# KristinnVikarJ/nbody-simulation

Measured on AMD Instinct MI355X. Metric: pair-interactions/sec + ms/step at N=1M direct O(N^2) (force + integration step), higher is better.
Workload: dtype f32; 1 GPU; direct O(N^2) f32, N=1048576 bodies, seeded 2-D Plummer sphere, masses 1, dt=0.1, clamp=0.001 (BASELINE.json configs[2]); n_bodies=1048576, targets_per_gpu=1048576, n_ranks=1, entry=one process per GPU (sharding.py over nbody_direct_{prep,run}_dev), exchange=none, arith=AUTO (FAST kernel; EXACT on hazardous positions)

## Files before the change

### nbody-simulation_amd/csrc/direct_kernels.h

```cpp
#pragma once
#include <hip/hip_runtime.h>
#include <stddef.h>
#include <stdint.h>

namespace nbody {

enum { kFlagHazard = 0, kFlagFallback = 1, kFlagNearCount = 2, kFlagState = 3 };

struct DirectArgs {
  const float2* pos_all;
  const float2* src_pos;
  const float* mass_all;
  int n_src;
  int tgt_begin;
  int n_tgt;
  float2* vel;
  float2* pos_out;
  float2* acc_out;
  float2* partial;
  int to_partial;
  float delta;
  float clamp;
  float uniform_mass;
  const int* flags;
  int run_state;
  const uint32_t* near_list;
  int src_couples;
  const float* src_minv;
  const float* tile_mass;
};

struct DirectConfig {
  int tpt = 1;
  int gsplit = 1;
  int use_asm = 4;
  bool nearfar = true;
};

struct NearFarLayout {
  size_t table_keys, table_bytes, is_near, scan, near_list, pos_far, minv_far, cub_temp, cub_temp_bytes, total;
};
NearFarLayout nearfar_layout(int64_t n_src);
constexpr int64_t kMaxMassClasses = 32;
constexpr int64_t kDirectTile = 1024;
constexpr float kFastBig = 1152921504606846976.0f;
constexpr float kFastTiny = 2.384185791015625e-07f;
constexpr int kFarPad = 16;
__host__ __device__ inline int64_t far_padded(int64_t n_slots) { return (n_slots + kFarPad - 1) / kFarPad * kFarPad; }
hipError_t launch_nearfar(hipStream_t s, const float2* pos, const float* mass, float heavy_base, int n, float clamp, int use_hazard,
                          int* flags, char* scratch, const NearFarLayout& L, const float2** pos_far, const uint32_t** near_list,
                          const uint32_t* rank = nullptr, const uint32_t* pad_slots = nullptr, int n_pad_slots = 0, bool couples = false,
                          const float** minv_far = nullptr);
hipError_t launch_decide_simple(hipStream_t s, int use_hazard, int* flags);

constexpr int kMutualSlice = 8192;
constexpr int kMutualStripItems = 256;
struct MutualArea {
  int n_slices;
  float2* tpart;
  float2* spart;
  float2* near_acc;
  const uint32_t* is_near;
  const uint32_t* near_scan;
};
int mutual_slices(int64_t n_slots);
size_t mutual_area_bytes(int64_t n_src);
MutualArea mutual_area(void* base, int64_t n_src, const uint32_t* is_near, const uint32_t* near_scan);
hipError_t launch_direct_mutual(hipStream_t s, const DirectArgs& a, const MutualArea& m);
hipError_t launch_direct_fast(hipStream_t s, const DirectArgs& a, const DirectConfig& c, bool noclamp);
hipError_t launch_direct_finish(hipStream_t s, const DirectArgs& a, int n_gsplit, bool add_near);
hipError_t launch_direct_exact(hipStream_t s, const DirectArgs& a);
hipError_t launch_hazard_scan(hipStream_t s, const float* xy, long n_floats, int* flags);
hipError_t launch_weights_to_mass(hipStream_t s, const uint32_t* w, float* m, long n);

}
```

### nbody-simulation_amd/csrc/direct_mutual.hip

```cpp
#include <hip/hip_runtime.h>
#include <stdint.h>

#include "direct_kernels.h"

namespace nbody {

namespace {

typedef float v2f __attribute__((ext_vector_type(2)));

constexpr int kWaves = 8;

constexpr int kSlice = kMutualSlice;
constexpr int kSliceCouples = kSlice / 2;
constexpr int kChunks = kSliceCouples / 64;
constexpr float kMarker = 1e30f;

__device__ __forceinline__ bool gate_open(const DirectArgs& a) { return a.run_state < 0 || a.flags[kFlagState] == a.run_state; }

__host__ __device__ inline int64_t off_items(int nb) { return (int64_t)nb * (nb - 1) / 2; }
__host__ __device__ inline int64_t item_of(int s, int b, int nb) { return (int64_t)s * nb - (int64_t)s * (s + 1) / 2 + (b - s - 1); }

__device__ __forceinline__ float4 couple_or_marker(const float4* c, int64_t k, int64_t n_couples) {
  return k < n_couples ? c[k] : make_float4(kMarker, kMarker, kMarker, kMarker);
}

#define NB_PX(K, H, D) "v_pk_add_f32 v[" D "], v[184:185], %[tx" #K "] op_sel:[0," #H "] op_sel_hi:[1," #H "] neg_lo:[0,1] neg_hi:[0,1]\n\t"
#define NB_PY(K, H, D) "v_pk_add_f32 v[" D "], v[186:187], %[ty" #K "] op_sel:[0," #H "] op_sel_hi:[1," #H "] neg_lo:[0,1] neg_hi:[0,1]\n\t"
#define NB_SQ(DX, DY, Q) "v_pk_mul_f32 v[" Q "], v[" DX "], v[" DX "]\n\tv_pk_fma_f32 v[" Q "], v[" DY "], v[" DY "], v[" Q "]\n\t"
#define NB_AD(XL, XH, YL, YH, SL, SH) "v_add_f32_e64 v" SL ", |v" XL "|, |v" YL "|\n\tv_add_f32_e64 v" SH ", |v" XH "|, |v" YH "|\n\t"
#define NB_DN(S, Q) "v_pk_fma_f32 v[" S "], v[" S "], v[" Q "], %[b]\n\t"
#define NB_RC(SL, SH) "v_rcp_f32_e32 v" SL ", v" SL "\n\tv_rcp_f32_e32 v" SH ", v" SH "\n\t"
#define NB_AC(T, DX, DY, S)                                                                                                          \
  "v_pk_fma_f32 %[ax" #T "], v[" DX "], v[" S "], %[ax" #T "]\n\t"                                                                    \
  "v_pk_fma_f32 v[188:189], v[" DX "], v[" S "], v[188:189] neg_lo:[1,0,0] neg_hi:[1,0,0]\n\t"                                                  \
  "v_pk_fma_f32 %[ay" #T "], v[" DY "], v[" S "], %[ay" #T "]\n\t"                                                                    \
  "v_pk_fma_f32 v[190:191], v[" DY "], v[" S "], v[190:191] neg_lo:[1,0,0] neg_hi:[1,0,0]\n\t"
#define NB_HALF(K0, K1, K2, K3, T0, T1, T2, T3, T4, T5, T6, T7)                                                                    \
  NB_PX(K0, 0, "192:193") NB_PX(K0, 1, "200:201") NB_PX(K1, 0, "208:209") NB_PX(K1, 1, "216:217")                                   \
  NB_PX(K2, 0, "224:225") NB_PX(K2, 1, "232:233") NB_PX(K3, 0, "240:241") NB_PX(K3, 1, "248:249")                                   \
  NB_PY(K0, 0, "194:195") NB_PY(K0, 1, "202:203") NB_PY(K1, 0, "210:211") NB_PY(K1, 1, "218:219")                                   \
  NB_PY(K2, 0, "226:227") NB_PY(K2, 1, "234:235") NB_PY(K3, 0, "242:243") NB_PY(K3, 1, "250:251")                                   \
  NB_SQ("192:193", "194:195", "196:197") NB_SQ("200:201", "202:203", "204:205") NB_SQ("208:209", "210:211", "212:213")             \
  NB_SQ("216:217", "218:219", "220:221") NB_SQ("224:225", "226:227", "228:229") NB_SQ("232:233", "234:235", "236:237")             \
  NB_SQ("240:241", "242:243", "244:245") NB_SQ("248:249", "250:251", "252:253")                                                    \
  "s_setprio 0\n\t"                                                                                                                \
  NB_AD("192", "193", "194", "195", "198", "199") NB_AD("200", "201", "202", "203", "206", "207")                                  \
  NB_AD("208", "209", "210", "211", "214", "215") NB_AD("216", "217", "218", "219", "222", "223")                                  \
  NB_AD("224", "225", "226", "227", "230", "231") NB_AD("232", "233", "234", "235", "238", "239")                                  \
  NB_AD("240", "241", "242", "243", "246", "247") NB_AD("248", "249", "250", "251", "254", "255")                                  \
  "s_setprio 1\n\t"                                                                                                                \
  NB_DN("198:199", "196:197") NB_DN("206:207", "204:205") NB_DN("214:215", "212:213") NB_DN("222:223", "220:221")                 \
  NB_DN("230:231", "228:229") NB_DN("238:239", "236:237") NB_DN("246:247", "244:245") NB_DN("254:255", "252:253")                 \
  NB_RC("198", "199")                                                                                                              \
  NB_RC("206", "207") NB_AC(T0, "192:193", "194:195", "198:199")                                                                   \
  NB_RC("214", "215") NB_AC(T1, "200:201", "202:203", "206:207")                                                                   \
  NB_RC("222", "223") NB_AC(T2, "208:209", "210:211", "214:215")                                                                   \
  NB_RC("230", "231") NB_AC(T3, "216:217", "218:219", "222:223")                                                                   \
  NB_RC("238", "239") NB_AC(T4, "224:225", "226:227", "230:231")                                                                   \
  NB_RC("246", "247") NB_AC(T5, "232:233", "234:235", "238:239")                                                                   \
  NB_RC("254", "255") NB_AC(T6, "240:241", "242:243", "246:247")                                                                   \
  NB_AC(T7, "248:249", "250:251", "254:255")
#define NB_ROT(R) "v_mov_b32_dpp " R ", " R " wave_ror:1 row_mask:0xf bank_mask:0xf\n\t"

__device__ __forceinline__ void mutual_chunk(const v2f* tx, const v2f* ty, v2f* ax, v2f* ay, float4 rc, float4& sacc,
                                             unsigned long long bias2) {
  asm volatile("v_mov_b32 v184, %[r0]\n\tv_mov_b32 v185, %[r1]\n\tv_mov_b32 v186, %[r2]\n\tv_mov_b32 v187, %[r3]\n\t"
               "v_mov_b32 v188, 0\n\tv_mov_b32 v189, 0\n\tv_mov_b32 v190, 0\n\tv_mov_b32 v191, 0\n\t"
               "s_mov_b32 s88, 64\n"
               ".Lnb_mutual_%=:\n\t"
               NB_HALF(0, 1, 2, 3, 0, 1, 2, 3, 4, 5, 6, 7) NB_HALF(4, 5, 6, 7, 8, 9, 10, 11, 12, 13, 14, 15)
               NB_ROT("v184") NB_ROT("v185") NB_ROT("v186") NB_ROT("v187") NB_ROT("v188") NB_ROT("v189") NB_ROT("v190") NB_ROT("v191")
               "s_sub_u32 s88, s88, 1\n\t"
               "s_cmp_lg_u32 s88, 0\n\t"
               "s_cbranch_scc1 .Lnb_mutual_%=\n\t"
               "v_mov_b32 %[o0], v188\n\tv_mov_b32 %[o1], v189\n\tv_mov_b32 %[o2], v190\n\tv_mov_b32 %[o3], v191\n\t"
               : [ax0] "+v"(ax[0]), [ax1] "+v"(ax[1]), [ax2] "+v"(ax[2]), [ax3] "+v"(ax[3]), [ax4] "+v"(ax[4]), [ax5] "+v"(ax[5]),
                 [ax6] "+v"(ax[6]), [ax7] "+v"(ax[7]), [ax8] "+v"(ax[8]), [ax9] "+v"(ax[9]), [ax10] "+v"(ax[10]), [ax11] "+v"(ax[11]),
                 [ax12] "+v"(ax[12]), [ax13] "+v"(ax[13]), [ax14] "+v"(ax[14]), [ax15] "+v"(ax[15]),
                 [ay0] "+v"(ay[0]), [ay1] "+v"(ay[1]), [ay2] "+v"(ay[2]), [ay3] "+v"(ay[3]), [ay4] "+v"(ay[4]), [ay5] "+v"(ay[5]),
                 [ay6] "+v"(ay[6]), [ay7] "+v"(ay[7]), [ay8] "+v"(ay[8]), [ay9] "+v"(ay[9]), [ay10] "+v"(ay[10]), [ay11] "+v"(ay[11]),
                 [ay12] "+v"(ay[12]), [ay13] "+v"(ay[13]), [ay14] "+v"(ay[14]), [ay15] "+v"(ay[15]),
                 [o0] "=&v"(sacc.x), [o1] "=&v"(sacc.y), [o2] "=&v"(sacc.z), [o3] "=&v"(sacc.w)
               : [tx0] "v"(tx[0]), [tx1] "v"(tx[1]), [tx2] "v"(tx[2]), [tx3] "v"(tx[3]), [tx4] "v"(tx[4]), [tx5] "v"(tx[5]),
                 [tx6] "v"(tx[6]), [tx7] "v"(tx[7]), [ty0] "v"(ty[0]), [ty1] "v"(ty[1]), [ty2] "v"(ty[2]), [ty3] "v"(ty[3]),
                 [ty4] "v"(ty[4]), [ty5] "v"(ty[5]), [ty6] "v"(ty[6]), [ty7] "v"(ty[7]), [b] "s"(bias2),
                 [r0] "v"(rc.x), [r1] "v"(rc.y), [r2] "v"(rc.z), [r3] "v"(rc.w)
               : "v184", "v185", "v186", "v187", "v188", "v189", "v190", "v191",
                 "v192", "v193", "v194", "v195", "v196", "v197", "v198", "v199", "v200", "v201", "v202", "v203", "v204", "v205",
                 "v206", "v207", "v208", "v209", "v210", "v211", "v212", "v213", "v214", "v215", "v216", "v217", "v218", "v219",
                 "v220", "v221", "v222", "v223", "v224", "v225", "v226", "v227", "v228", "v229", "v230", "v231", "v232", "v233",
                 "v234", "v235", "v236", "v237", "v238", "v239", "v240", "v241", "v242", "v243", "v244", "v245", "v246", "v247",
                 "v248", "v249", "v250", "v251", "v252", "v253", "v254", "v255", "s88", "scc");
}
#undef NB_PX
#undef NB_PY
#undef NB_SQ
#undef NB_AD
#undef NB_DN
#undef NB_RC
#undef NB_AC
#undef NB_HALF
#undef NB_ROT

__global__ __launch_bounds__(kWaves * 64) void direct_mutual(const DirectArgs a, MutualArea m, int64_t lo) {
  if (!gate_open(a)) return;
  const int nb = m.n_slices;
  const int64_t n_off = off_items(nb);
  const int64_t item = lo + blockIdx.x;
  int s, b;
  if (item < n_off) {
    s = 0;
    int64_t first = 0;
    while (first + (nb - 1 - s) <= item) first += nb - 1 - s++;
    b = s + 1 + (int)(item - first);
  } else {
    s = b = (int)(item - n_off);
  }
  const bool diag = s == b;
  const int lane = threadIdx.x & 63;
  const int w = __builtin_amdgcn_readfirstlane((int)(threadIdx.x >> 6));
  const float4* couples = reinterpret_cast<const float4*>(a.src_pos);
  const int64_t n_couples = a.n_src / 2;
  v2f tx[8], ty[8];
  const int64_t tc0 = (int64_t)s * kSliceCouples + 512 * w + 8 * lane;
#pragma unroll
  for (int k = 0; k < 8; ++k) {
    const float4 c = couple_or_marker(couples, tc0 + k, n_couples);
    tx[k] = v2f{c.x, c.y};
    ty[k] = v2f{c.z, c.w};
  }
  float tot_x[16], tot_y[16];
#pragma unroll
  for (int t = 0; t < 16; ++t) tot_x[t] = tot_y[t] = 0.f;
  const unsigned long long bias2 = 0x1280000012800000ull;
  __shared__ float4 red[2][kWaves][64];
  float* spart = reinterpret_cast<float*>(m.spart + (size_t)blockIdx.x * kSlice);
  __builtin_amdgcn_s_setprio(1);
  for (int c = 0; c < kChunks; ++c) {
    const float4 rc = couple_or_marker(couples, (int64_t)b * kSliceCouples + 64 * c + lane, n_couples);
    v2f ax[16], ay[16];
#pragma unroll
    for (int t = 0; t < 16; ++t) ax[t] = ay[t] = v2f{0.f, 0.f};
    float4 sacc;
    mutual_chunk(tx, ty, ax, ay, rc, sacc, bias2);
#pragma unroll
    for (int t = 0; t < 16; ++t) {
      tot_x[t] += ax[t].x + ax[t].y;
      tot_y[t] += ay[t].x + ay[t].y;
    }
    if (diag) continue;
    red[c & 1][w][lane] = sacc;
    __syncthreads();
    if (threadIdx.x < 256) {
      const int q = threadIdx.x >> 2, comp = threadIdx.x & 3;
      float r = 0.f;
#pragma unroll
      for (int v = 0; v < kWaves; ++v) r += reinterpret_cast<const float*>(&red[c & 1][v][q])[comp];
      spart[(size_t)(128 * c + 2 * q + (comp & 1)) * 2 + (comp >> 1)] = r;
    }
  }
  float2* tpart = m.tpart + (size_t)blockIdx.x * kSlice;
#pragma unroll
  for (int t = 0; t < 16; ++t) tpart[1024 * w + 16 * lane + t] = make_float2(tot_x[t], tot_y[t]);
}

__global__ __launch_bounds__(256) void direct_mutual_near(const DirectArgs a, MutualArea m) {
  if (!gate_open(a)) return;
  const int n_near = a.flags[kFlagNearCount];
  const float4* couples = reinterpret_cast<const float4*>(a.src_pos);
  const int n_couples = a.n_src / 2;
  __shared__ float2 red[256];
  for (int k = blockIdx.x; k < n_near; k += gridDim.x) {
    const float2 p = a.pos_all[a.near_list[k]];
    float ax = 0.f, ay = 0.f;
    for (int q = threadIdx.x; q < n_couples; q += 256) {
      const float4 c = couples[q];
#pragma unroll
      for (int h = 0; h < 2; ++h) {
        const float dx = (h ? c.y : c.x) - p.x, dy = (h ? c.w : c.z) - p.y;
        const float sum = __builtin_fabsf(dx) + __builtin_fabsf(dy);
        const float d2 = __builtin_fmaf(dy, dy, dx * dx);
        const float s = __builtin_amdgcn_rcpf(__builtin_fmaf(sum, d2, 8.0779356694631609e-28f));
        ax = __builtin_fmaf(dx, s, ax);
        ay = __builtin_fmaf(dy, s, ay);
      }
    }
    red[threadIdx.x] = make_float2(ax, ay);
    __syncthreads();
    for (int w = 128; w > 0; w >>= 1) {
      if ((int)threadIdx.x < w) {
        red[threadIdx.x].x += red[threadIdx.x + w].x;
        red[threadIdx.x].y += red[threadIdx.x + w].y;
      }
      __syncthreads();
    }
    if (threadIdx.x == 0) m.near_acc[k] = red[0];
    __syncthreads();
  }
}

__global__ __launch_bounds__(256) void direct_mutual_reduce(const DirectArgs a, MutualArea m, int64_t lo, int64_t hi, int first, int last) {
  if (!gate_open(a)) return;
  const int i = blockIdx.x * 256 + threadIdx.x;
  if (i >= a.n_tgt) return;
  const int nb = m.n_slices;
  const int s = i / kSlice, l = i % kSlice;
  int r0 = 0, r1 = s;
  while (r0 < r1) {
    const int mid = (r0 + r1) >> 1;
    if (item_of(mid, s, nb) < lo) r0 = mid + 1; else r1 = mid;
  }
  const int64_t b0 = s + 1 < nb ? item_of(s, s + 1, nb) : 0, b1 = s + 1 < nb ? item_of(s, nb - 1, nb) + 1 : 0;
  const int64_t d = off_items(nb) + s;
  const bool touched = (r0 < s && item_of(r0, s, nb) < hi) || (b0 < hi && b1 > lo) || (d >= lo && d < hi);
  if (!touched && !first && !last) return;
  float2 acc = first ? make_float2(0.f, 0.f) : a.partial[i];
  for (int r = r0; r < s; ++r) {
    const int64_t it = item_of(r, s, nb);
    if (it >= hi) break;
    const float2 p = m.spart[(size_t)(it - lo) * kSlice + l];
    acc.x += p.x;
    acc.y += p.y;
  }
  {
    for (int64_t it = b0 > lo ? b0 : lo; it < (b1 < hi ? b1 : hi); ++it) {
      const float2 p = m.tpart[(size_t)(it - lo) * kSlice + l];
      acc.x += p.x;
      acc.y += p.y;
    }
  }
  if (d >= lo && d < hi) {
    const float2 p = m.tpart[(size_t)(d - lo) * kSlice + l];
    acc.x += p.x;
    acc.y += p.y;
  }
  if (last) {
    if (m.is_near[i]) acc = m.near_acc[m.near_scan[i]];
    acc = make_float2(acc.x * a.uniform_mass, acc.y * a.uniform_mass);
  }
  a.partial[i] = acc;
}

}

int mutual_slices(int64_t n_slots) { return (int)((n_slots + kSlice - 1) / kSlice); }

size_t mutual_area_bytes(int64_t n_src) {
  return 2 * (size_t)kMutualStripItems * kSlice * sizeof(float2) + ((size_t)n_src / 64 + 2) * sizeof(float2);
}

MutualArea mutual_area(void* base, int64_t n_src, const uint32_t* is_near, const uint32_t* near_scan) {
  MutualArea m{};
  m.n_slices = mutual_slices(far_padded(n_src));
  float2* p = (float2*)base;
  m.tpart = p;
  p += (size_t)kMutualStripItems * kSlice;
  m.spart = p;
  p += (size_t)kMutualStripItems * kSlice;
  m.near_acc = p;
  m.is_near = is_near;
  m.near_scan = near_scan;
  return m;
}

hipError_t launch_direct_mutual(hipStream_t s, const DirectArgs& a, const MutualArea& m) {
  if (a.n_tgt <= 0) return hipSuccess;
  if (!a.src_couples || a.tgt_begin != 0 || a.n_src < a.n_tgt || m.n_slices != mutual_slices(a.n_src)) return hipErrorInvalidValue;
  const int64_t items = off_items(m.n_slices) + m.n_slices;
  const dim3 rgrid((unsigned)((a.n_tgt + 255) / 256));
  hipLaunchKernelGGL(direct_mutual_near, dim3(256), dim3(256), 0, s, a, m);
  for (int64_t lo = 0; lo < items; lo += kMutualStripItems) {
    const int64_t hi = lo + kMutualStripItems < items ? lo + kMutualStripItems : items;
    hipLaunchKernelGGL(direct_mutual, dim3((unsigned)(hi - lo)), dim3(kWaves * 64), 0, s, a, m, lo);
    hipLaunchKernelGGL(direct_mutual_reduce, rgrid, dim3(256), 0, s, a, m, lo, hi, lo == 0 ? 1 : 0, hi == items ? 1 : 0);
  }
  return hipGetLastError();
}

}
```

Baseline: 9596 billion pair-interactions/s.

## Exploit symmetry in diagonal mutual tiles and split near-body pass across sources

Measured after the change: 9931 billion pair-interactions/s, median of 6. 1.03x the previous value.

```diff
diff --git a/nbody-simulation_amd/csrc/direct_kernels.h b/nbody-simulation_amd/csrc/direct_kernels.h
--- a/nbody-simulation_amd/csrc/direct_kernels.h
+++ b/nbody-simulation_amd/csrc/direct_kernels.h
@@ -55,11 +55,13 @@
 
 constexpr int kMutualSlice = 8192;
 constexpr int kMutualStripItems = 256;
+constexpr int kMutualNearSplit = 32;
+constexpr int kMutualNearRows = 64;
 struct MutualArea {
   int n_slices;
   float2* tpart;
   float2* spart;
-  float2* near_acc;
+  float2* near_part;
   const uint32_t* is_near;
   const uint32_t* near_scan;
 };
diff --git a/nbody-simulation_amd/csrc/direct_mutual.hip b/nbody-simulation_amd/csrc/direct_mutual.hip
--- a/nbody-simulation_amd/csrc/direct_mutual.hip
+++ b/nbody-simulation_amd/csrc/direct_mutual.hip
@@ -2,6 +2,7 @@
 #include <stdint.h>
 
 #include "direct_kernels.h"
+#include "mutual_schedule.h"
 
 namespace nbody {
 
@@ -17,9 +18,6 @@
 constexpr float kMarker = 1e30f;
 
 __device__ __forceinline__ bool gate_open(const DirectArgs& a) { return a.run_state < 0 || a.flags[kFlagState] == a.run_state; }
-
-__host__ __device__ inline int64_t off_items(int nb) { return (int64_t)nb * (nb - 1) / 2; }
-__host__ __device__ inline int64_t item_of(int s, int b, int nb) { return (int64_t)s * nb - (int64_t)s * (s + 1) / 2 + (b - s - 1); }
 
 __device__ __forceinline__ float4 couple_or_marker(const float4* c, int64_t k, int64_t n_couples) {
   return k < n_couples ? c[k] : make_float4(kMarker, kMarker, kMarker, kMarker);
@@ -63,11 +61,11 @@
   NB_AC(T7, "248:249", "250:251", "254:255")
 #define NB_ROT(R) "v_mov_b32_dpp " R ", " R " wave_ror:1 row_mask:0xf bank_mask:0xf\n\t"
 
-__device__ __forceinline__ void mutual_chunk(const v2f* tx, const v2f* ty, v2f* ax, v2f* ay, float4 rc, float4& sacc,
+__device__ __forceinline__ void mutual_steps(const v2f* tx, const v2f* ty, v2f* ax, v2f* ay, float4& rc, float4& sacc, int steps,
                                              unsigned long long bias2) {
   asm volatile("v_mov_b32 v184, %[r0]\n\tv_mov_b32 v185, %[r1]\n\tv_mov_b32 v186, %[r2]\n\tv_mov_b32 v187, %[r3]\n\t"
-               "v_mov_b32 v188, 0\n\tv_mov_b32 v189, 0\n\tv_mov_b32 v190, 0\n\tv_mov_b32 v191, 0\n\t"
-               "s_mov_b32 s88, 64\n"
+               "v_mov_b32 v188, %[o0]\n\tv_mov_b32 v189, %[o1]\n\tv_mov_b32 v190, %[o2]\n\tv_mov_b32 v191, %[o3]\n\t"
+               "s_mov_b32 s88, %[n]\n"
                ".Lnb_mutual_%=:\n\t"
                NB_HALF(0, 1, 2, 3, 0, 1, 2, 3, 4, 5, 6, 7) NB_HALF(4, 5, 6, 7, 8, 9, 10, 11, 12, 13, 14, 15)
                NB_ROT("v184") NB_ROT("v185") NB_ROT("v186") NB_ROT("v187") NB_ROT("v188") NB_ROT("v189") NB_ROT("v190") NB_ROT("v191")
@@ -75,17 +73,18 @@
                "s_cmp_lg_u32 s88, 0\n\t"
                "s_cbranch_scc1 .Lnb_mutual_%=\n\t"
                "v_mov_b32 %[o0], v188\n\tv_mov_b32 %[o1], v189\n\tv_mov_b32 %[o2], v190\n\tv_mov_b32 %[o3], v191\n\t"
+               "v_mov_b32 %[r0], v184\n\tv_mov_b32 %[r1], v185\n\tv_mov_b32 %[r2], v186\n\tv_mov_b32 %[r3], v187\n\t"
                : [ax0] "+v"(ax[0]), [ax1] "+v"(ax[1]), [ax2] "+v"(ax[2]), [ax3] "+v"(ax[3]), [ax4] "+v"(ax[4]), [ax5] "+v"(ax[5]),
                  [ax6] "+v"(ax[6]), [ax7] "+v"(ax[7]), [ax8] "+v"(ax[8]), [ax9] "+v"(ax[9]), [ax10] "+v"(ax[10]), [ax11] "+v"(ax[11]),
                  [ax12] "+v"(ax[12]), [ax13] "+v"(ax[13]), [ax14] "+v"(ax[14]), [ax15] "+v"(ax[15]),
                  [ay0] "+v"(ay[0]), [ay1] "+v"(ay[1]), [ay2] "+v"(ay[2]), [ay3] "+v"(ay[3]), [ay4] "+v"(ay[4]), [ay5] "+v"(ay[5]),
                  [ay6] "+v"(ay[6]), [ay7] "+v"(ay[7]), [ay8] "+v"(ay[8]), [ay9] "+v"(ay[9]), [ay10] "+v"(ay[10]), [ay11] "+v"(ay[11]),
                  [ay12] "+v"(ay[12]), [ay13] "+v"(ay[13]), [ay14] "+v"(ay[14]), [ay15] "+v"(ay[15]),
-                 [o0] "=&v"(sacc.x), [o1] "=&v"(sacc.y), [o2] "=&v"(sacc.z), [o3] "=&v"(sacc.w)
+                 [o0] "+v"(sacc.x), [o1] "+v"(sacc.y), [o2] "+v"(sacc.z), [o3] "+v"(sacc.w),
+                 [r0] "+v"(rc.x), [r1] "+v"(rc.y), [r2] "+v"(rc.z), [r3] "+v"(rc.w)
                : [tx0] "v"(tx[0]), [tx1] "v"(tx[1]), [tx2] "v"(tx[2]), [tx3] "v"(tx[3]), [tx4] "v"(tx[4]), [tx5] "v"(tx[5]),
                  [tx6] "v"(tx[6]), [tx7] "v"(tx[7]), [ty0] "v"(ty[0]), [ty1] "v"(ty[1]), [ty2] "v"(ty[2]), [ty3] "v"(ty[3]),
-                 [ty4] "v"(ty[4]), [ty5] "v"(ty[5]), [ty6] "v"(ty[6]), [ty7] "v"(ty[7]), [b] "s"(bias2),
-                 [r0] "v"(rc.x), [r1] "v"(rc.y), [r2] "v"(rc.z), [r3] "v"(rc.w)
+                 [ty4] "v"(ty[4]), [ty5] "v"(ty[5]), [ty6] "v"(ty[6]), [ty7] "v"(ty[7]), [b] "s"(bias2), [n] "s"(steps)
                : "v184", "v185", "v186", "v187", "v188", "v189", "v190", "v191",
                  "v192", "v193", "v194", "v195", "v196", "v197", "v198", "v199", "v200", "v201", "v202", "v203", "v204", "v205",
                  "v206", "v207", "v208", "v209", "v210", "v211", "v212", "v213", "v214", "v215", "v216", "v217", "v218", "v219",
@@ -103,26 +102,7 @@
 #undef NB_HALF
 #undef NB_ROT
 
-__global__ __launch_bounds__(kWaves * 64) void direct_mutual(const DirectArgs a, MutualArea m, int64_t lo) {
-  if (!gate_open(a)) return;
-  const int nb = m.n_slices;
-  const int64_t n_off = off_items(nb);
-  const int64_t item = lo + blockIdx.x;
-  int s, b;
-  if (item < n_off) {
-    s = 0;
-    int64_t first = 0;
-    while (first + (nb - 1 - s) <= item) first += nb - 1 - s++;
-    b = s + 1 + (int)(item - first);
-  } else {
-    s = b = (int)(item - n_off);
-  }
-  const bool diag = s == b;
-  const int lane = threadIdx.x & 63;
-  const int w = __builtin_amdgcn_readfirstlane((int)(threadIdx.x >> 6));
-  const float4* couples = reinterpret_cast<const float4*>(a.src_pos);
-  const int64_t n_couples = a.n_src / 2;
-  v2f tx[8], ty[8];
+__device__ __forceinline__ void load_targets(const float4* couples, int64_t n_couples, int s, int w, int lane, v2f* tx, v2f* ty) {
   const int64_t tc0 = (int64_t)s * kSliceCouples + 512 * w + 8 * lane;
 #pragma unroll
   for (int k = 0; k < 8; ++k) {
@@ -130,26 +110,38 @@
     tx[k] = v2f{c.x, c.y};
     ty[k] = v2f{c.z, c.w};
   }
+}
+
+__device__ __forceinline__ void zero_acc(v2f* ax, v2f* ay) {
+#pragma unroll
+  for (int t = 0; t < 16; ++t) ax[t] = ay[t] = v2f{0.f, 0.f};
+}
+
+__device__ __forceinline__ void add_chunk(const v2f* ax, const v2f* ay, float* tot_x, float* tot_y) {
+#pragma unroll
+  for (int t = 0; t < 16; ++t) {
+    tot_x[t] += ax[t].x + ax[t].y;
+    tot_y[t] += ay[t].x + ay[t].y;
+  }
+}
+
+constexpr unsigned long long kBias2 = 0x1280000012800000ull;
+
+__device__ __forceinline__ void off_item(const float4* couples, int64_t n_couples, int s, int b, int w, int lane, float4 (*red)[kWaves][64],
+                                         float2* tpart, float2* spart_f2) {
+  v2f tx[8], ty[8];
+  load_targets(couples, n_couples, s, w, lane, tx, ty);
   float tot_x[16], tot_y[16];
 #pragma unroll
   for (int t = 0; t < 16; ++t) tot_x[t] = tot_y[t] = 0.f;
-  const unsigned long long bias2 = 0x1280000012800000ull;
-  __shared__ float4 red[2][kWaves][64];
-  float* spart = reinterpret_cast<float*>(m.spart + (size_t)blockIdx.x * kSlice);
-  __builtin_amdgcn_s_setprio(1);
+  float* spart = reinterpret_cast<float*>(spart_f2);
   for (int c = 0; c < kChunks; ++c) {
-    const float4 rc = couple_or_marker(couples, (int64_t)b * kSliceCouples + 64 * c + lane, n_couples);
+    float4 rc = couple_or_marker(couples, (int64_t)b * kSliceCouples + 64 * c + lane, n_couples);
     v2f ax[16], ay[16];
-#pragma unroll
-    for (int t = 0; t < 16; ++t) ax[t] = ay[t] = v2f{0.f, 0.f};
-    float4 sacc;
-    mutual_chunk(tx, ty, ax, ay, rc, sacc, bias2);
-#pragma unroll
-    for (int t = 0; t < 16; ++t) {
-      tot_x[t] += ax[t].x + ax[t].y;
-      tot_y[t] += ay[t].x + ay[t].y;
-    }
-    if (diag) continue;
+    zero_acc(ax, ay);
+    float4 sacc = make_float4(0.f, 0.f, 0.f, 0.f);
+    mutual_steps(tx, ty, ax, ay, rc, sacc, 64, kBias2);
+    add_chunk(ax, ay, tot_x, tot_y);
     red[c & 1][w][lane] = sacc;
     __syncthreads();
     if (threadIdx.x < 256) {
@@ -160,9 +152,83 @@
       spart[(size_t)(128 * c + 2 * q + (comp & 1)) * 2 + (comp >> 1)] = r;
     }
   }
+#pragma unroll
+  for (int t = 0; t < 16; ++t) tpart[1024 * w + 16 * lane + t] = make_float2(tot_x[t], tot_y[t]);
+}
+
+__device__ __forceinline__ void diag_item(const float4* couples, int64_t n_couples, int s, int w, int lane, float4 (*src)[8][64],
+                                          float2* out) {
+  using namespace mutual_schedule;
+  v2f tx[8], ty[8];
+  load_targets(couples, n_couples, s, w, lane, tx, ty);
+  float tot_x[16], tot_y[16];
+#pragma unroll
+  for (int t = 0; t < 16; ++t) tot_x[t] = tot_y[t] = 0.f;
+  const int64_t c0 = (int64_t)s * kSliceCouples;
+  for (int p = 0; p < kDiagPhases; ++p) {
+    const int u = diag_block(w, p), r0 = diag_first_step(w, p), n = diag_steps(p);
+    for (int j = 0; j < 8; ++j) {
+      float4 rc = couple_or_marker(couples, c0 + 512 * u + 8 * ((lane - r0) & 63) + j, n_couples);
+      v2f ax[16], ay[16];
+      zero_acc(ax, ay);
+      float4 sacc = make_float4(0.f, 0.f, 0.f, 0.f);
+      int moved;
+      if (p == 0) {
+        mutual_steps(tx, ty, ax, ay, rc, sacc, 1, kBias2);
+        sacc = make_float4(0.f, 0.f, 0.f, 0.f);
+        mutual_steps(tx, ty, ax, ay, rc, sacc, n - 2, kBias2);
+        const float4 keep = sacc;
+        mutual_steps(tx, ty, ax, ay, rc, sacc, 1, kBias2);
+        sacc = keep;
+        moved = n - 1;
+      } else {
+        mutual_steps(tx, ty, ax, ay, rc, sacc, n, kBias2);
+        moved = n;
+      }
+      add_chunk(ax, ay, tot_x, tot_y);
+      const int shift = (r0 + moved) & 63;
+      if (shift) {
+        const int from = (lane + shift) & 63;
+        sacc = make_float4(__shfl(sacc.x, from), __shfl(sacc.y, from), __shfl(sacc.z, from), __shfl(sacc.w, from));
+      }
+      float4& d = src[u][j][lane];
+      if (p == 0) {
+        d = sacc;
+      } else {
+        const float4 o = d;
+        d = make_float4(o.x + sacc.x, o.y + sacc.y, o.z + sacc.z, o.w + sacc.w);
+      }
+    }
+    __syncthreads();
+  }
+#pragma unroll
+  for (int k = 0; k < 8; ++k) {
+    const float4 q = src[w][k][lane];
+    out[1024 * w + 16 * lane + 2 * k] = make_float2(tot_x[2 * k] + q.x, tot_y[2 * k] + q.z);
+    out[1024 * w + 16 * lane + 2 * k + 1] = make_float2(tot_x[2 * k + 1] + q.y, tot_y[2 * k + 1] + q.w);
+  }
+  __syncthreads();
+}
+
+__global__ __launch_bounds__(kWaves * 64) void direct_mutual(const DirectArgs a, MutualArea m, int64_t lo) {
+  if (!gate_open(a)) return;
+  const int nb = m.n_slices;
+  int s, b;
+  mutual_schedule::unit_slices(lo + blockIdx.x, nb, s, b);
+  const int lane = threadIdx.x & 63;
+  const int w = __builtin_amdgcn_readfirstlane((int)(threadIdx.x >> 6));
+  const float4* couples = reinterpret_cast<const float4*>(a.src_pos);
+  const int64_t n_couples = a.n_src / 2;
   float2* tpart = m.tpart + (size_t)blockIdx.x * kSlice;
-#pragma unroll
-  for (int t = 0; t < 16; ++t) tpart[1024 * w + 16 * lane + t] = make_float2(tot_x[t], tot_y[t]);
+  float2* spart = m.spart + (size_t)blockIdx.x * kSlice;
+  __shared__ float4 lds[8][8][64];
+  __builtin_amdgcn_s_setprio(1);
+  if (s < b) {
+    off_item(couples, n_couples, s, b, w, lane, reinterpret_cast<float4(*)[kWaves][64]>(&lds[0][0][0]), tpart, spart);
+  } else {
+    diag_item(couples, n_couples, s, w, lane, lds, tpart);
+    if (s + 1 < nb) diag_item(couples, n_couples, s + 1, w, lane, lds, spart);
+  }
 }
 
 __global__ __launch_bounds__(256) void direct_mutual_near(const DirectArgs a, MutualArea m) {
@@ -170,11 +236,14 @@
   const int n_near = a.flags[kFlagNearCount];
   const float4* couples = reinterpret_cast<const float4*>(a.src_pos);
   const int n_couples = a.n_src / 2;
+  const int per = (n_couples + kMutualNearSplit - 1) / kMutualNearSplit;
+  const int q0 = blockIdx.x * per, q1 = q0 + per < n_couples ? q0 + per : n_couples;
   __shared__ float2 red[256];
-  for (int k = blockIdx.x; k < n_near; k += gridDim.x) {
+  for (int k = blockIdx.y; k < n_near; k += gridDim.y) {
     const float2 p = a.pos_all[a.near_list[k]];
     float ax = 0.f, ay = 0.f;
-    for (int q = threadIdx.x; q < n_couples; q += 256) {
+#pragma unroll 4
+    for (int q = q0 + (int)threadIdx.x; q < q1; q += 256) {
       const float4 c = couples[q];
 #pragma unroll
       for (int h = 0; h < 2; ++h) {
@@ -195,12 +264,13 @@
       }
       __syncthreads();
     }
-    if (threadIdx.x == 0) m.near_acc[k] = red[0];
+    if (threadIdx.x == 0) m.near_part[(size_t)k * kMutualNearSplit + blockIdx.x] = red[0];
     __syncthreads();
   }
 }
 
 __global__ __launch_bounds__(256) void direct_mutual_reduce(const DirectArgs a, MutualArea m, int64_t lo, int64_t hi, int first, int last) {
+  using mutual_schedule::item_of;
   if (!gate_open(a)) return;
   const int i = blockIdx.x * 256 + threadIdx.x;
   if (i >= a.n_tgt) return;
@@ -211,32 +281,44 @@
     const int mid = (r0 + r1) >> 1;
     if (item_of(mid, s, nb) < lo) r0 = mid + 1; else r1 = mid;
   }
+  int re = s;
+  r1 = r0;
+  while (r1 < re) {
+    const int mid = (r1 + re) >> 1;
+    if (item_of(mid, s, nb) < hi) r1 = mid + 1; else re = mid;
+  }
   const int64_t b0 = s + 1 < nb ? item_of(s, s + 1, nb) : 0, b1 = s + 1 < nb ? item_of(s, nb - 1, nb) + 1 : 0;
-  const int64_t d = off_items(nb) + s;
-  const bool touched = (r0 < s && item_of(r0, s, nb) < hi) || (b0 < hi && b1 > lo) || (d >= lo && d < hi);
-  if (!touched && !first && !last) return;
+  const int64_t w0 = b0 > lo ? b0 : lo, w1 = b1 < hi ? b1 : hi;
+  const int64_t d = mutual_schedule::diag_unit(s, nb);
+  const bool has_d = d >= lo && d < hi;
+  if (r0 == r1 && w0 >= w1 && !has_d && !first && !last) return;
   float2 acc = first ? make_float2(0.f, 0.f) : a.partial[i];
-  for (int r = r0; r < s; ++r) {
-    const int64_t it = item_of(r, s, nb);
-    if (it >= hi) break;
-    const float2 p = m.spart[(size_t)(it - lo) * kSlice + l];
+#pragma unroll 8
+  for (int r = r0; r < r1; ++r) {
+    const float2 p = m.spart[(size_t)(item_of(r, s, nb) - lo) * kSlice + l];
     acc.x += p.x;
     acc.y += p.y;
   }
-  {
-    for (int64_t it = b0 > lo ? b0 : lo; it < (b1 < hi ? b1 : hi); ++it) {
-      const float2 p = m.tpart[(size_t)(it - lo) * kSlice + l];
-      acc.x += p.x;
-      acc.y += p.y;
-    }
-  }
-  if (d >= lo && d < hi) {
-    const float2 p = m.tpart[(size_t)(d - lo) * kSlice + l];
+#pragma unroll 8
+  for (int64_t it = w0; it < w1; ++it) {
+    const float2 p = m.tpart[(size_t)(it - lo) * kSlice + l];
     acc.x += p.x;
     acc.y += p.y;
   }
+  if (has_d) {
+    const float2 p = ((s & 1) ? m.spart : m.tpart)[(size_t)(d - lo) * kSlice + l];
+    acc.x += p.x;
+    acc.y += p.y;
+  }
   if (last) {
-    if (m.is_near[i]) acc = m.near_acc[m.near_scan[i]];
+    if (m.is_near[i]) {
+      const float2* np = m.near_part + (size_t)m.near_scan[i] * kMutualNearSplit;
+      acc = np[0];
+      for (int g = 1; g < kMutualNearSplit; ++g) {
+        acc.x += np[g].x;
+        acc.y += np[g].y;
+      }
+    }
     acc = make_float2(acc.x * a.uniform_mass, acc.y * a.uniform_mass);
   }
   a.partial[i] = acc;
@@ -247,7 +329,7 @@
 int mutual_slices(int64_t n_slots) { return (int)((n_slots + kSlice - 1) / kSlice); }
 
 size_t mutual_area_bytes(int64_t n_src) {
-  return 2 * (size_t)kMutualStripItems * kSlice * sizeof(float2) + ((size_t)n_src / 64 + 2) * sizeof(float2);
+  return 2 * (size_t)kMutualStripItems * kSlice * sizeof(float2) + ((size_t)n_src / 64 + 2) * kMutualNearSplit * sizeof(float2);
 }
 
 MutualArea mutual_area(void* base, int64_t n_src, const uint32_t* is_near, const uint32_t* near_scan) {
@@ -258,7 +340,7 @@
   p += (size_t)kMutualStripItems * kSlice;
   m.spart = p;
   p += (size_t)kMutualStripItems * kSlice;
-  m.near_acc = p;
+  m.near_part = p;
   m.is_near = is_near;
   m.near_scan = near_scan;
   return m;
@@ -267,13 +349,19 @@
 hipError_t launch_direct_mutual(hipStream_t s, const DirectArgs& a, const MutualArea& m) {
   if (a.n_tgt <= 0) return hipSuccess;
   if (!a.src_couples || a.tgt_begin != 0 || a.n_src < a.n_tgt || m.n_slices != mutual_slices(a.n_src)) return hipErrorInvalidValue;
-  const int64_t items = off_items(m.n_slices) + m.n_slices;
+  int dev = 0, cus = 0;
+  hipError_t e = hipGetDevice(&dev);
+  if (e == hipSuccess) e = hipDeviceGetAttribute(&cus, hipDeviceAttributeMultiprocessorCount, dev);
+  if (e != hipSuccess) return e;
+  if (cus <= 0) return hipErrorInvalidValue;
+  const int64_t units = mutual_schedule::units(m.n_slices);
+  const int64_t strip = mutual_schedule::strip_units(cus, kMutualStripItems);
   const dim3 rgrid((unsigned)((a.n_tgt + 255) / 256));
-  hipLaunchKernelGGL(direct_mutual_near, dim3(256), dim3(256), 0, s, a, m);
-  for (int64_t lo = 0; lo < items; lo += kMutualStripItems) {
-    const int64_t hi = lo + kMutualStripItems < items ? lo + kMutualStripItems : items;
+  hipLaunchKernelGGL(direct_mutual_near, dim3(kMutualNearSplit, kMutualNearRows), dim3(256), 0, s, a, m);
+  for (int64_t lo = 0; lo < units; lo += strip) {
+    const int64_t hi = lo + strip < units ? lo + strip : units;
     hipLaunchKernelGGL(direct_mutual, dim3((unsigned)(hi - lo)), dim3(kWaves * 64), 0, s, a, m, lo);
-    hipLaunchKernelGGL(direct_mutual_reduce, rgrid, dim3(256), 0, s, a, m, lo, hi, lo == 0 ? 1 : 0, hi == items ? 1 : 0);
+    hipLaunchKernelGGL(direct_mutual_reduce, rgrid, dim3(256), 0, s, a, m, lo, hi, lo == 0 ? 1 : 0, hi == units ? 1 : 0);
   }
   return hipGetLastError();
 }
diff --git a/nbody-simulation_amd/csrc/mutual_schedule.h b/nbody-simulation_amd/csrc/mutual_schedule.h
--- /dev/null
+++ b/nbody-simulation_amd/csrc/mutual_schedule.h
@@ -0,0 +1,40 @@
+#pragma once
+#include <stdint.h>
+
+#if defined(__HIPCC__)
+#define NB_HD __host__ __device__
+#else
+#define NB_HD
+#endif
+
+namespace nbody {
+namespace mutual_schedule {
+
+NB_HD inline int64_t off_items(int nb) { return (int64_t)nb * (nb - 1) / 2; }
+NB_HD inline int64_t item_of(int s, int b, int nb) { return (int64_t)s * nb - (int64_t)s * (s + 1) / 2 + (b - s - 1); }
+NB_HD inline int64_t units(int nb) { return off_items(nb) + (nb + 1) / 2; }
+NB_HD inline void unit_slices(int64_t unit, int nb, int& s, int& b) {
+  const int64_t n_off = off_items(nb);
+  if (unit < n_off) {
+    s = 0;
+    int64_t first = 0;
+    while (first + (nb - 1 - s) <= unit) first += nb - 1 - s++;
+    b = s + 1 + (int)(unit - first);
+  } else {
+    s = b = 2 * (int)(unit - n_off);
+  }
+}
+NB_HD inline int64_t diag_unit(int s, int nb) { return off_items(nb) + s / 2; }
+
+NB_HD inline int strip_units(int cus, int capacity) { return cus >= capacity ? capacity : capacity / cus * cus; }
+
+constexpr int kDiagPhases = 5;
+NB_HD inline int diag_block(int w, int p) { return (w + p) & 7; }
+NB_HD inline int diag_first_step(int w, int p) { return p == 4 && w >= 4 ? 1 : 0; }
+NB_HD inline int diag_steps(int p) { return p == 0 ? 33 : p == 4 ? 32 : 64; }
+NB_HD inline bool diag_one_sided(int p, int i) { return p == 0 && (i == 0 || i == 32); }
+
+}
+}
+
+#undef NB_HD
```
